# dmjovan/NeRF-Workspaces-Explorer

Measured on AMD Instinct MI355X. Metric: ray-samples/sec (800x800, 192 samples, 8x256 MLP), higher is better.
Workload: dtype f16x3 (split-fp16 MFMA, fp32 accumulate)

## Files before the change

include/nwe.h:

```cpp
#ifndef NWE_H
#define NWE_H

#include <stdint.h>

#ifdef __cplusplus
extern "C" {
#endif

typedef struct nwe_ctx nwe_ctx;

enum {
    NWE_OK = 0,
    NWE_ERR_INVALID = 1,
    NWE_ERR_UNSUPPORTED = 2,
    NWE_ERR_HIP = 3,
    NWE_ERR_STATE = 4
};

enum { NWE_NET_COARSE = 0, NWE_NET_FINE = 1 };

enum {
    NWE_PREC_F16X3 = 0,
    NWE_PREC_F16X1 = 1,
    NWE_PREC_F32 = 2
// ... 60 lines not shown

int nwe_to8b(nwe_ctx *ctx, const float *rgb_dev, uint8_t *out_dev, int64_t n, void *stream);

int64_t nwe_flops_per_eval(const nwe_ctx *ctx, int which);

float nwe_last_kernel_ms(nwe_ctx *ctx);

int nwe_last_launch_parts(nwe_ctx *ctx, float *ms2, int64_t *rays2);


int64_t nwe_packed_bytes(const nwe_ctx *ctx, int which);
int nwe_packed_copy(const nwe_ctx *ctx, int which, void *host_dst, int64_t bytes);
int64_t nwe_packed_bias_count(const nwe_ctx *ctx, int which);
int nwe_packed_bias_copy(const nwe_ctx *ctx, int which, float *host_dst, int64_t count);
float nwe_packed_scale(const nwe_ctx *ctx, int which);

int nwe_debug_set_fine_depths(nwe_ctx *ctx, const float *z_dev);

int nwe_debug_set_raw(nwe_ctx *ctx, const float *raw_coarse_dev, const float *raw_fine_dev);
int nwe_debug_set_coarse_weights(nwe_ctx *ctx, const float *weights_dev);

int nwe_debug_set_fold(nwe_ctx *ctx, int on);

int nwe_set_white_background(nwe_ctx *ctx, int on);

int nwe_set_train_tables(nwe_ctx *ctx, const float *t_rand_dev, const float *noise_coarse_dev, const float *noise_fine_dev,
                         const float *u_sorted_dev);

int nwe_debug_set_decomposition(nwe_ctx *ctx, int mode);
int nwe_debug_last_plan(const nwe_ctx *ctx);
// ... 10 lines not shown
```

nerf-workspaces-explorer_amd/_lib.py:

```python
from __future__ import annotations

import ctypes as C
import os

_HERE = os.path.dirname(os.path.abspath(__file__))
LIB_PATH = os.environ.get("NWE_LIB") or os.path.join(_HERE, "libnwe_hip.so")

NWE_OK, NWE_ERR_INVALID, NWE_ERR_UNSUPPORTED, NWE_ERR_HIP, NWE_ERR_STATE = 0, 1, 2, 3, 4
NET_COARSE, NET_FINE = 0, 1
PREC_F16X3, PREC_F16X1, PREC_F32 = 0, 1, 2
PRECISIONS = {"f16x3": PREC_F16X3, "f16x1": PREC_F16X1, "f32": PREC_F32}

OUTPUT_FIELDS = ("rgb", "depth", "acc", "disp", "z_std", "rgb_coarse", "depth_coarse", "acc_coarse", "disp_coarse",
                 "raw_coarse", "raw_fine", "z_fine", "weights_coarse", "sample_cond", "sample_amp", "sample_switch", "feat_map", "flags")

SYMBOLS = ("nwe_create", "nwe_destroy", "nwe_last_error", "nwe_set_network", "nwe_set_sampling", "nwe_render", "nwe_render_tiled",
           "nwe_create_rays", "nwe_render_rays", "nwe_to8b", "nwe_flops_per_eval", "nwe_last_kernel_ms", "nwe_packed_bytes",
           "nwe_packed_copy", "nwe_packed_bias_count", "nwe_packed_bias_copy", "nwe_packed_scale",
           "nwe_debug_set_fine_depths", "nwe_debug_set_raw", "nwe_debug_set_coarse_weights", "nwe_debug_set_fold", "nwe_set_train_tables", "nwe_set_white_background", "nwe_debug_set_decomposition", "nwe_debug_last_plan", "nwe_debug_set_stamps", "nwe_selftest",
           "nwe_last_warning", "nwe_debug_peer_access", "nwe_set_network_no_view_dirs", "nwe_last_launch_parts")


class Outputs(C.Structure):
    _fields_ = [("struct_bytes", C.c_uint64)] + [(name, C.c_void_p) for name in OUTPUT_FIELDS]

    def __init__(self, **kw):
        super().__init__(struct_bytes=C.sizeof(Outputs), **kw)


_lib = None


def build_hint() -> str:
# ... 17 lines not shown
        "nwe_set_network_no_view_dirs": (I, [P, I, I, I, I, I, I, C.POINTER(P), C.POINTER(P)]),
        "nwe_set_sampling": (I, [P, P, P, I, P, I]),
        "nwe_render": (I, [P, P, I, I, I, F, F, F, F, F, F, I, I, I, C.POINTER(Outputs), P]),
        "nwe_render_tiled": (I, [C.POINTER(P), I, P, I, I, I, F, F, F, F, F, F, I, P, P, P, P, P]),
        "nwe_create_rays": (I, [P, P, I, I, I, F, F, F, F, F, F, I, I, P, P]),
        "nwe_render_rays": (I, [P, P, I64, I, C.POINTER(Outputs), P]),
        "nwe_to8b": (I, [P, P, P, I64, P]),
        "nwe_flops_per_eval": (I64, [P, I]),
        "nwe_last_kernel_ms": (F, [P]),
        "nwe_last_launch_parts": (I, [P, C.POINTER(F), C.POINTER(I64)]),
        "nwe_packed_bytes": (I64, [P, I]),
        "nwe_packed_copy": (I, [P, I, P, I64]),
        "nwe_packed_bias_count": (I64, [P, I]),
        "nwe_packed_bias_copy": (I, [P, I, P, I64]),
        "nwe_packed_scale": (F, [P, I]),
        "nwe_debug_set_fine_depths": (I, [P, P]),
        "nwe_debug_set_raw": (I, [P, P, P]),
        "nwe_debug_set_coarse_weights": (I, [P, P]),
        "nwe_debug_set_fold": (I, [P, I]),
        "nwe_set_train_tables": (I, [P, P, P, P, P]),
        "nwe_set_white_background": (I, [P, I]),
        "nwe_debug_set_decomposition": (I, [P, I]),
        "nwe_debug_last_plan": (I, [P]),
        "nwe_debug_set_stamps": (I, [P, P]),
        "nwe_selftest": (I, [P, C.POINTER(C.c_int32)]),
        "nwe_last_warning": (C.c_char_p, [P]),
        "nwe_debug_peer_access": (I, [P, P]),
    }
    for name, (res, args) in sig.items():
        fn = getattr(lib, name)
# ... 4 lines not shown
```

nerf-workspaces-explorer_amd/csrc/nwe_abi.hip:

```cpp
#include <algorithm>
#include <cmath>
#include <cstdlib>
#include <cstring>
#include <string>
#include <vector>

#include "nwe_host.h"

using namespace nwe;

namespace {

struct NetState {
    bool set = false;
    int D = 0, W = 0, in_xyz = 0, in_dir = 0, skip = -1;
    int out_ch = 0;
    int64_t flops = 0;
    std::vector<float> blob;
    NetF32 f32 = {};
    float* d_blob = nullptr;
    bool mfma_ok = false;
    int form = kFormFolded;
    std::vector<uint8_t> stream;
    std::vector<float> bias_tab;
    int n_chunks = 0;
    float w_scale = 1.f;
    NetMfma mf = {};
    uint8_t* d_stream = nullptr;
    float* d_bias = nullptr;
};

thread_local std::string g_create_error;

}

struct nwe_ctx {
    int device = -1;
    bool host_only = false;
    NetState net[2];
    float *d_t = nullptr, *d_omt = nullptr, *d_u = nullptr;
    int ns = 0, ni = 0;
// ... 103 lines not shown
}

template <class T>
void put_chunk(NetState& n, const T* w, const T* b, int ld, const RowMap& rows, int rt, const std::vector<Segment>& segs) {
    for (int i = 0; i < 32; ++i) { const int r = rows(rt, i); n.bias_tab.push_back(r >= 0 ? (float)b[r] : 0.f); }
    for (const Segment& sg : segs)
        for (int s = 0; s < sg.ksteps; ++s) put_tile_pair(n.stream, w, ld, rows, rt, sg, s, n.w_scale);
}

void pack_mfma(NetState& n, const float* const* w, const float* const* b) {
    const int D = n.D, W = n.W, KH = W / 16;
    const int iv = D, ife = D + 1, ia = D + 2, irgb = D + 3;
    const bool folded = n.form == kFormFolded, noview = n.form == kFormNoViewDirs;
    n.stream.clear();
    n.bias_tab.clear();
    std::vector<double> wv, bv;
    if (folded) {
        const int ldv = W + n.in_dir;
        wv.assign((size_t)(W / 2) * ldv, 0.0);
        bv.assign(W / 2, 0.0);
        for (int r = 0; r < W / 2; ++r) {
            const float* vr = w[iv] + (size_t)r * ldv;
            double* o = wv.data() + (size_t)r * ldv;
            double acc_b = (double)b[iv][r];
            for (int k = 0; k < W; ++k) {
                const double vk = (double)vr[k];
                const float* fr = w[ife] + (size_t)k * W;
                for (int c = 0; c < W; ++c) o[c] += vk * (double)fr[c];
                acc_b += vk * (double)b[ife][k];
            }
// ... 19 lines not shown
    };
    layer(0, W, n.in_xyz, W / 32, 0, {{1, 4, 0}});
    for (int i = 1; i < D; ++i) {
        if (i == n.skip + 1) layer(i, W, W + n.in_xyz, W / 32, 0, {{1, 4, 0}, {0, KH, n.in_xyz}});
        else layer(i, W, W, W / 32, 0, {{0, KH, 0}});
    }
    if (noview) {
        layer(D, 4, W, 1, 1, {{0, KH, 0}});
        n.n_chunks = (int)(n.bias_tab.size() / 32);
        return;
    }
    if (!folded) {
        layer(ife, W, W, W / 32, 0, {{0, KH, 0}});
        layer(ia, 1, W, 1, 1, {{0, KH, 0}});
    }
    if (folded) {
        RowMap rows{W / 2, 0};
        for (int rt = 0; rt < W / 64; ++rt) put_chunk(n, wv.data(), bv.data(), W + n.in_dir, rows, rt, {{0, KH, 0}, {2, 2, W}});
    } else {
        layer(iv, W / 2, W + n.in_dir, W / 64, 0, {{0, KH, 0}, {2, 2, W}});
    }
    layer(irgb, 3, W / 2, 1, 1, {{0, KH / 2, 0}});
    n.n_chunks = (int)(n.bias_tab.size() / 32);
    if (folded) {
        for (int k = 0; k < W; ++k) n.bias_tab.push_back(w[ia][k]);
        n.bias_tab.push_back(b[ia][0]);
        n.bias_tab.resize(n.bias_tab.size() + 31, 0.f);
    }
}

void pack_f32(NetState& n, const float* const* w, const float* const* b) {
    n.blob.clear();
    auto add = [&](int li, int K, int N) {
        LayerF32 L; L.K = K; L.N = N; L.wt_off = (int64_t)n.blob.size();
        n.blob.resize(n.blob.size() + (size_t)K * N);
        float* wt = n.blob.data() + L.wt_off;
        for (int k = 0; k < K; ++k) for (int o = 0; o < N; ++o) wt[(size_t)k * N + o] = w[li][(size_t)o * K + k];
        L.b_off = (int64_t)n.blob.size();
        n.blob.insert(n.blob.end(), b[li], b[li] + N);
// ... 208 lines not shown
    for (int i = 0; i < n_layers; ++i)
        if (!w[i] || !b[i]) return fail(c, NWE_ERR_INVALID, "null weight or bias pointer");
    NetState& n = c->net[which];
    n.set = false;
    n.D = depth; n.W = width; n.in_xyz = in_xyz; n.in_dir = in_dir; n.skip = skip_layer; n.out_ch = out_ch;
    n.flops = algo_flops(n);
    pack_f32(n, w, b);
    n.form = in_dir == 0 ? kFormNoViewDirs : (c->fold != 0 ? kFormFolded : kFormReference);
    n.mfma_ok = mfma_supported(depth, width, in_xyz, in_dir, skip_layer, n.form);
    if (n.mfma_ok) pack_mfma(n, w, b); else { n.stream.clear(); n.bias_tab.clear(); n.n_chunks = 0; }
    n.mf = {};
    n.mf.D = depth; n.mf.W = width; n.mf.skip = skip_layer; n.mf.form = n.form;
    n.mf.n_tiles = (int)(n.stream.size() / kTileBytes);
    n.mf.n_chunks = n.mfma_ok ? n.n_chunks : 0;
    n.mf.inv_scale = 1.f / n.w_scale;
    if (!c->host_only) {
        DeviceGuard guard;
        HIPCHK(c, hipSetDevice(c->device));
        { const int rc = wait_for_launches(c); if (rc) return rc; }
        if (n.d_blob) { (void)hipFree(n.d_blob); n.d_blob = nullptr; }
        if (n.d_stream) { (void)hipFree(n.d_stream); n.d_stream = nullptr; }
        if (n.d_bias) { (void)hipFree(n.d_bias); n.d_bias = nullptr; }
        HIPCHK(c, hipMalloc(&n.d_blob, n.blob.size() * sizeof(float)));
        HIPCHK(c, hipMemcpy(n.d_blob, n.blob.data(), n.blob.size() * sizeof(float), hipMemcpyHostToDevice));
        if (n.mfma_ok) {
            HIPCHK(c, hipMalloc(&n.d_stream, n.stream.size()));
            HIPCHK(c, hipMemcpy(n.d_stream, n.stream.data(), n.stream.size(), hipMemcpyHostToDevice));
            HIPCHK(c, hipMalloc(&n.d_bias, n.bias_tab.size() * sizeof(float)));
            HIPCHK(c, hipMemcpy(n.d_bias, n.bias_tab.data(), n.bias_tab.size() * sizeof(float), hipMemcpyHostToDevice));
        }
// ... 291 lines not shown
    return (int64_t)c->net[which].bias_tab.size();
}

int nwe_packed_bias_copy(const nwe_ctx* c, int which, float* host_dst, int64_t count) {
    if (!c || which < 0 || which > 1 || !host_dst || !c->net[which].set) return NWE_ERR_INVALID;
    if (count != (int64_t)c->net[which].bias_tab.size()) return NWE_ERR_INVALID;
    std::memcpy(host_dst, c->net[which].bias_tab.data(), (size_t)count * sizeof(float));
    return NWE_OK;
}

float nwe_packed_scale(const nwe_ctx* c, int which) {
    if (!c || which < 0 || which > 1 || !c->net[which].set) return 0.f;
    return c->net[which].w_scale;
}

int nwe_debug_set_fine_depths(nwe_ctx* c, const float* z_dev) {
    if (!c) return NWE_ERR_INVALID;
    c->dbg_z_fine = z_dev;
    return NWE_OK;
}

int nwe_debug_set_raw(nwe_ctx* c, const float* raw_coarse_dev, const float* raw_fine_dev) {
    if (!c) return NWE_ERR_INVALID;
    c->dbg_raw_c = raw_coarse_dev; c->dbg_raw_f = raw_fine_dev;
    return NWE_OK;
}

int nwe_debug_set_coarse_weights(nwe_ctx* c, const float* weights_dev) {
    if (!c) return NWE_ERR_INVALID;
    c->dbg_w = weights_dev;
// ... 59 lines not shown
```

nerf-workspaces-explorer_amd/csrc/nwe_host.h:

```cpp
#pragma once
#include <hip/hip_runtime.h>
#include <stdint.h>

#include "nwe_device.h"

namespace nwe {

struct LayerF32 {
    int K, N;
    int64_t wt_off, b_off;
};
struct NetF32 {
    const float* blob;
    int D, W, in_xyz, in_dir, skip;
    LayerF32 pts[16];
    LayerF32 views, feature, alpha, rgb;
    LayerF32 output;
    int out_ch;
};
constexpr int kMaxDepth = 16;

void launch_render_f32(const RenderArgs& a, const NetF32& nc, const NetF32& nf, hipStream_t stream);

struct NetMfma {
    const uint8_t* stream;
    const float* bias;
    int n_tiles, n_chunks;
    float inv_scale;
    int D, W, skip;
    int form;
};

enum Form {
    kFormReference = 0,
    kFormFolded = 1,
    kFormNoViewDirs = 2
};

bool mfma_supported(int D, int W, int in_xyz, int in_dir, int skip, int form);
struct LaunchInfo {
    hipEvent_t mid = nullptr;
    int plan = -1;
    int64_t rays_first = 0;
    bool mid_recorded = false;
};
// ... 10 lines not shown
```

nerf-workspaces-explorer_amd/csrc/nwe_mfma_kernels.h:

```cpp
#pragma once
#include "nwe_host.h"

namespace nwe {

typedef _Float16 h8 __attribute__((ext_vector_type(8)));
typedef float f16v __attribute__((ext_vector_type(16)));

#define LDS_AS __attribute__((address_space(3)))

constexpr int kWaves = 4;
constexpr int kRaysPerWave = 32;

template <int W, int D>
struct Shape {
    static constexpr int NT = W / 32;
    static constexpr int KH = W / 16;
    static constexpr int KG = 4;
    static constexpr int KD = 2;
    static constexpr int NTV = W / 64;
    static constexpr int KV = W / 32;
    static constexpr int N_L0 = 2 * KG / kWaves;
    static constexpr int N_H = 2 * KH / kWaves;
    static constexpr int N_S = 2 * (KH + KG) / kWaves;
    static constexpr int N_V = 2 * (KH + KD) / kWaves;
// ... 189 lines not shown
    const char* buf0;
    const char* tail0;
    int t3;
    uint32_t blk_dst_tail;
    int tail_first;
    const float* bias_tab;
    int chunk;
    int b;
    int wave;
    uint32_t lane_off;
    const uint8_t* blk_src;
    uint32_t blk_dst;
    bool skip_lo = false;
#ifdef NWE_STAMPS
    unsigned long long st_pre = 0, st_wait = 0, st_post = 0, st_t0 = 0;
#endif

    __device__ __forceinline__ void start(const uint8_t* s, const float* bias) {
        stream = s; bias_tab = bias; next_tile = 0; chunk = 0; b = 0; t3 = 0;
    }
    __device__ __forceinline__ const char* cur() const { return buf0 + b * CHUNK_BYTES; }
    __device__ __forceinline__ const char* next() const { return buf0 + (b ^ 1) * CHUNK_BYTES; }
    __device__ __forceinline__ const char* tail() const { return tail0 + t3 * (2 * kTileBytes); }
    __device__ __forceinline__ void begin(int n_per_wave, int buffer, int ahead) {
        blk_src = stream + ((size_t)next_tile + (size_t)wave * n_per_wave) * kTileBytes;
        blk_dst = lds_chunks + buffer * CHUNK_BYTES + wave * n_per_wave * kTileBytes;
        next_tile += n_per_wave * kWaves;
        skip_lo = !X3 && (n_per_wave & 1) == 0;
        if (X3) {
            int slot = t3 + ahead;
// ... 346 lines not shown
            const _Float16 hh = (_Float16)v;
            Ehi[s][j] = hh;
            Elo[s][j] = X3 ? (_Float16)(v - (float)hh) : (_Float16)0.f;
        }
    }
}

template <int W, int D, bool X3>
struct ViewDma {
    using S = Shape<W, D>;
    static constexpr int nb(int rt) { return rt + 1 < S::NTV ? S::N_V : S::N_RGB; }
    static constexpr int na(int rt) { return rt + 2 < S::NTV ? S::N_V : (rt + 2 == S::NTV ? S::N_RGB : 0); }
    using Plan0 = EpiPlan<X3, S::KH, S::KH + S::KD, true, DmaPlan<nb(0), na(0), S::KH + S::KD>::mask()>;
};

template <int RT, int W, int D, bool X3, bool SIGMA_TILE, class WalkerT>
__device__ __forceinline__ void view_tiles(WalkerT& wk, Frags& F, int lane, h8* Ahi, h8* Alo, const h8* GDhi,
                                           const h8* GDlo, h8* Bhi, h8* Blo, Pend& P0, Pend& P1, float inv_scale,
                                           const float* dot_tab = nullptr, float* dot = nullptr) {
    using S = Shape<W, D>;
    constexpr int par = SIGMA_TILE ? (RT + 1) & 1 : RT & 1;
    Pend& cur = par ? P1 : P0;
    Pend& prev = par ? P0 : P1;
    constexpr int PH = (RT * (S::KH + S::KD)) % (PD + 1);
    constexpr int NB = ViewDma<W, D, X3>::nb(RT);
    constexpr int NA = ViewDma<W, D, X3>::na(RT);
    if constexpr (RT == 0 && SIGMA_TILE) {
        h8 d0, d1, d2, d3;
        tile_mma<0, S::KH, S::KD, PH, X3, false, NB, NA, true>(wk, F, lane, false, false, false, nullptr, nullptr, Ahi, Alo, GDhi, GDlo, cur,
                                                               prev, inv_scale, 0.f, d0, d1, d2, d3);
    } else if constexpr (RT == 0) {
        constexpr int L = 2 * S::NT - 2;
        tile_mma<0, S::KH, S::KD, PH, X3, true, NB, NA, true, true, true>(wk, F, lane, false, false, false, nullptr, nullptr, Ahi, Alo, GDhi, GDlo,
                                                                          cur, prev, inv_scale, 0.f, Ahi[L], Alo[L], Ahi[L + 1], Alo[L + 1], -1,
                                                                          dot_tab + (S::NT - 1) * 32, dot);
    } else {
        tile_mma<0, S::KH, S::KD, PH, X3, true, NB, NA, true>(wk, F, lane, false, false, false, nullptr, nullptr, Ahi, Alo, GDhi, GDlo, cur,
                                                              prev, inv_scale, 0.f, Bhi[2 * RT - 2], Blo[2 * RT - 2], Bhi[2 * RT - 1],
                                                              Blo[2 * RT - 1]);
    }
    if constexpr (RT + 1 < S::NTV) view_tiles<RT + 1, W, D, X3, SIGMA_TILE>(wk, F, lane, Ahi, Alo, GDhi, GDlo, Bhi, Blo, P0, P1, inv_scale);
}

#ifndef NWE_COARSE_DENSITY_ONLY
#define NWE_COARSE_DENSITY_ONLY 1
#endif
template <int D, int SKIP>
constexpr bool density_only_built(int form) {
    return NWE_COARSE_DENSITY_ONLY != 0 && form == kFormFolded && !(SKIP >= 0 && SKIP / 2 == D / 2 - 1);
}

template <int W, int D, int SKIP, bool X3, int FORM, class WalkerT>
__device__ __forceinline__ void mlp_eval(WalkerT& wk, Frags& F, int lane, float inv_scale, h8* Ghi, h8* Glo, const char* gd_lds,
                                         const float* dot_tab, bool density_only, float& o_r, float& o_g, float& o_b, float& o_s) {
    using S = Shape<W, D>;
    static_assert(D % 2 == 0, "trunk depth must be even");
    static_assert(SKIP < 0 || SKIP % 2 == 0, "skip layer index must be even");
    static_assert(S::NT % 2 == 0 && S::NTV % 2 == 0, "tile counts must be even");
    constexpr bool FOLD = FORM == kFormFolded, NOVIEW = FORM == kFormNoViewDirs;
    h8 Ahi[S::KH], Alo[S::KH], Bhi[S::KH], Blo[S::KH];
    Pend P0, P1;
    constexpr int NPAIR = D / 2;
    constexpr int SKIP_PAIR = SKIP < 0 ? -1 : SKIP / 2;

    layer<S::NT, 0, S::KG, X3, false, S::N_H, true>(wk, F, lane, false, SKIP_PAIR == 0, nullptr, nullptr, Ghi, Glo, Ahi, Alo, P0, P1,
                                                    inv_scale, 0.f, 0.f);
    auto pair_body = [&](bool use_g, bool skip_next, bool last) __attribute__((always_inline)) {
        layer<S::NT, S::KG, S::KH, X3, true, S::N_H, false>(wk, F, lane, use_g, false, Ghi, Glo, Ahi, Alo, Bhi, Blo, P0, P1, inv_scale,
                                                            0.f, 0.f);
// ... 7 lines not shown
#endif
    if constexpr (NWE_PEEL_SKIP != 0 && SKIP_PAIR >= 0 && SKIP_PAIR < PAIRS) {
#pragma unroll 1
        for (int pair = 0; pair < SKIP_PAIR; ++pair) pair_body(false, pair + 1 == SKIP_PAIR, false);
        pair_body(true, false, SKIP_PAIR == NPAIR - 1);
#pragma unroll 1
        for (int pair = SKIP_PAIR + 1; pair < PAIRS; ++pair) pair_body(false, false, pair == NPAIR - 1);
    } else {
#pragma unroll 1
        for (int pair = 0; pair < PAIRS; ++pair) {
            const bool last = pair == NPAIR - 1;
            pair_body(pair == SKIP_PAIR, !last && pair + 1 == SKIP_PAIR, last);
        }
    }
    float sig = 0.f;
    auto sigma_of = [&]() __attribute__((always_inline)) { return __fadd_rn(__fadd_rn(sig, __shfl_xor(sig, 32, 64)), dot_tab[S::NT * 32]); };
    if constexpr (FOLD) {
        constexpr bool G_LAST = SKIP_PAIR == NPAIR - 1;
        if constexpr (density_only_built<D, SKIP>(FORM)) {
            if (density_only) {
                using TrunkA = EpiPlan<X3, S::KH, S::KH, false, DmaPlan<S::N_H, S::N_V, S::KH>::mask()>;
                using TrunkA0 = EpiPlan<X3, S::KH, S::KH, false, DmaPlan<S::N_H, 0, S::KH>::mask()>;
                using TrunkB = EpiPlan<X3, S::KH, S::KH, false, DmaPlan<S::N_V, S::N_V, S::KH>::mask()>;
                using TrunkB0 = EpiPlan<X3, S::KH, S::KH, false, DmaPlan<0, 0, S::KH>::mask()>;
                static_assert(TrunkA::NG == TrunkA0::NG && TrunkB::NG == TrunkB0::NG,
                              "the last trunk tiles must run the epilogues they carry in the full evaluation's order (dot FMAs)");
                static_assert(!G_LAST, "density_only_built: the last trunk layer takes no gamma(x) k-steps here");
                layer<S::NT, 0, S::KH, X3, true, 0, false, true, 0, false>(wk, F, lane, false, false, nullptr, nullptr, Ahi, Alo, Bhi, Blo, P0, P1,
                                                                           inv_scale, 0.f, 0.f, -1, dot_tab, &sig);
                drain_dot<typename ViewDma<W, D, X3>::Plan0, X3>(P1, inv_scale, dot_tab + (S::NT - 1) * 32 + 4 * (lane >> 5), sig);
                o_s = sigma_of();
// ... 14 lines not shown
                                                              P1, inv_scale, 0.f, Bhi[L], Blo[L], Bhi[L + 1], Blo[L + 1]);
        o_r = pend_value(P0, 0, inv_scale);
        o_g = pend_value(P0, 1, inv_scale);
        o_b = pend_value(P0, 2, inv_scale);
        o_s = pend_value(P0, 3, inv_scale);
        return;
    }
    static_assert((S::NTV * (S::KH + S::KD)) % (PD + 1) == 0, "the view tiles must restore the ring phase");
    h8 GDhi[S::KD], GDlo[S::KD];
#pragma unroll
    for (int k = 0; k < S::KD; ++k) {
        GDhi[k] = *reinterpret_cast<const h8*>(gd_lds + (2 * k) * kTileBytes);
        if (X3) GDlo[k] = *reinterpret_cast<const h8*>(gd_lds + (2 * k + 1) * kTileBytes);
    }
    if constexpr (FOLD) {
        view_tiles<0, W, D, X3, false>(wk, F, lane, Bhi, Blo, GDhi, GDlo, Ahi, Alo, P0, P1, inv_scale, dot_tab, &sig);
        const float sigma = sigma_of();
        tile_mma<0, S::KV, 0, 0, X3, true, 0, 0, false, true>(wk, F, lane, false, false, false, nullptr, nullptr, Ahi, Alo, nullptr, nullptr, P0,
                                                              P1, inv_scale, 0.f, Ahi[LV], Alo[LV], Ahi[LV + 1], Alo[LV + 1]);
        o_s = sigma;
        o_r = pend_value(P0, 0, inv_scale);
        o_g = pend_value(P0, 1, inv_scale);
        o_b = pend_value(P0, 2, inv_scale);
        return;
    } else {
        tile_mma<0, S::KH, 0, 0, X3, true, S::N_V, S::N_V, true>(wk, F, lane, false, false, false, nullptr, nullptr, Bhi, Blo, nullptr, nullptr,
                                                                 P0, P1, inv_scale, -INFINITY, Ahi[L], Alo[L], Ahi[L + 1], Alo[L + 1]);
        const float sigma = pend_value(P0, 0, inv_scale);
        view_tiles<0, W, D, X3, true>(wk, F, lane, Ahi, Alo, GDhi, GDlo, Bhi, Blo, P0, P1, inv_scale);
        tile_mma<0, S::KV, 0, 0, X3, true, 0, 0, false, true>(wk, F, lane, false, false, false, nullptr, nullptr, Bhi, Blo, nullptr, nullptr, P1,
                                                              P0, inv_scale, 0.f, Bhi[LV], Blo[LV], Bhi[LV + 1], Blo[LV + 1]);
        o_s = sigma;
// ... 10 lines not shown
struct Smem {
    using S = Shape<W, D>;
    static constexpr int WBYTES = (SPLIT ? kSplitMaxSamples : kWaves * kPacketMaxSamples) * kRaysPerWave * 4;
    static constexpr int CHUNKS = 2 * S::CHUNK_BYTES;
    static constexpr int BOFF = CHUNKS;
    static constexpr int BIAS_BYTES = ((S::N_CHUNKS * 32 * 4 + 255) / 256) * 256;
    static constexpr int WOFF = BOFF + 2 * BIAS_BYTES;
    static constexpr int TOFF = WOFF + WBYTES;
    static constexpr int XOFF = TOFF + (2 * kMaxSamples + kMaxImportance) * 4;
    static constexpr int LOFF = XOFF + (SPLIT ? 2 * kWaves * kRaysPerWave * 16 : 0);
    static constexpr int GOFF = LOFF + 3 * 2 * kTileBytes;
    static constexpr int TOTAL = GOFF + kWaves * 2 * S::KD * kTileBytes;
    static_assert(XOFF % 16 == 0 && LOFF % 16 == 0 && GOFF % 16 == 0 && TOTAL <= 160 * 1024, "LDS budget");
};

__host__ __device__ inline bool is_lean(const RenderArgs& a) {
    const nwe_outputs& o = a.out;
    return !o.raw_coarse && !o.raw_fine && !o.z_fine && !o.weights_coarse && !o.disp && !o.z_std && !o.rgb_coarse && !o.depth_coarse &&
           !o.acc_coarse && !o.disp_coarse && !o.sample_cond && !o.sample_amp && !o.sample_switch && !o.feat_map && !a.z_fine_in && !a.raw_in_c &&
           !a.raw_in_f && !a.w_in && !a.t_rand && !a.noise_c && !a.noise_f && !a.u_rand && !a.stamps && !a.rays;
}

template <int W, int D, int SKIP, bool X3, bool SPLIT, int FORM, bool LEAN>
__global__ void __launch_bounds__(256) render_mfma_kernel(RenderArgs a_in, NetMfma nc, NetMfma nf) {
    RenderArgs a = a_in;
    if constexpr (LEAN) {
        a.out.raw_coarse = a.out.raw_fine = a.out.z_fine = a.out.weights_coarse = nullptr;
        a.out.disp = a.out.z_std = a.out.rgb_coarse = a.out.depth_coarse = a.out.acc_coarse = a.out.disp_coarse = nullptr;
        a.out.sample_cond = a.out.sample_amp = a.out.sample_switch = a.out.feat_map = nullptr;
        a.z_fine_in = a.raw_in_c = a.raw_in_f = a.w_in = a.t_rand = a.noise_c = a.noise_f = a.u_rand = nullptr;
        a.stamps = nullptr; a.rays = nullptr;
    }
    using S = Shape<W, D>;
    using SM = Smem<W, D, SPLIT>;
    __shared__ __attribute__((aligned(16))) char smem[SM::TOTAL];

    const int lane = threadIdx.x & 63;
    const int wave = __builtin_amdgcn_readfirstlane(threadIdx.x >> 6);
    const int half = lane >> 5;
    const int ns = a.n_samples, ni = a.n_importance;
// ... 19 lines not shown
    const int row = (int)(ridx64 < a.n_rays ? ridx64 : a.n_rays - 1);
    const int64_t ridx = row, rclamp = row;
    const RaySeed seed = seed_ray(a, rclamp);
    auto fresh_ray = [&]() __attribute__((always_inline)) {
        RaySeed sd = seed;
        asm volatile("" : "+v"(sd.pose), "+v"(sd.x), "+v"(sd.y));
        return make_ray<false>(a, sd);
    };

    Walker<S::CHUNK_BYTES, X3> wk;
    wk.buf0 = smem; wk.lds_chunks = (uint32_t)(uintptr_t)(LDS_AS char*)smem;
    wk.tail0 = smem + SM::LOFF; wk.lds_tail = wk.lds_chunks + SM::LOFF; wk.t3 = 0;
    wk.b = 0; wk.wave = wave; wk.lane_off = lane * 16;

    char* gd_lds = smem + SM::GOFF + wave * (2 * S::KD * kTileBytes) + lane * 16;
    if constexpr (FORM != kFormNoViewDirs) {
        const Ray rv = make_ray<true>(a, seed);
        h8 GDhi[S::KD], GDlo[S::KD];
        encode<2, S::KD, X3>(rv.vx, rv.vy, rv.vz, half, GDhi, GDlo);
#pragma unroll
        for (int k = 0; k < S::KD; ++k) {
            *reinterpret_cast<h8*>(gd_lds + (2 * k) * kTileBytes) = GDhi[k];
            *reinterpret_cast<h8*>(gd_lds + (2 * k + 1) * kTileBytes) = GDlo[k];
        }
    }

    FineSampler fs;
    fs.wc = reinterpret_cast<float*>(smem + SM::WOFF) + (SPLIT ? 0 : wave * (kPacketMaxSamples * kRaysPerWave)) + (lane & 31);
    const bool wc_writer = !SPLIT || wave == 0;
    fs.stride = kRaysPerWave; fs.u_tab = s_u; fs.ns = ns; fs.ni = ni;
    fs.cd.t_tab = s_t; fs.cd.omt_tab = s_omt; fs.cd.ns = ns;
    fs.cd.jitter = a.t_rand; fs.cd.row = row;
    fs.u_rand = a.u_rand;
    __syncthreads();

    Composite comp;
    uint32_t flags = 0;
#ifdef NWE_STAMPS
    unsigned long long st_enc = 0, st_sync = 0, st_mlp = 0, st_comp = 0;
    const unsigned long long st_begin = __builtin_amdgcn_s_memtime();
    const unsigned long long st_real = __builtin_amdgcn_s_memrealtime();
#endif
    for (int pass = 0; pass < (ni > 0 ? 2 : 1); ++pass) {
        const NetMfma& net = pass == 0 ? nc : nf;
        const float* bias = s_bias + (pass == 0 ? 0 : SM::BIAS_BYTES / 4);
        const float* dot_tab = bias + NCH * 32;
        const int Stot = pass == 0 ? ns : ns + ni;
        const bool density_only = LEAN && density_only_built<D, SKIP>(FORM) && pass == 0 && ni > 0;
        const float* noise = pass == 0 ? a.noise_c : a.noise_f;
        const float* raw_in = pass == 0 ? a.raw_in_c : a.raw_in_f;
        if (pass == 0 && a.w_in) {
            if (wc_writer) for (int s = 0; s < ns; ++s) fs.wc[s * kRaysPerWave] = a.w_in[rclamp * ns + s];
            continue;
        }
        comp.reset();
        if constexpr (SPLIT) {
            int produced = 0;
            auto gen = [&](const Ray& ray) -> float {
                const int i = produced++;
                if (i >= Stot) return 0.f;
                if (pass == 0) return fs.cd.z(ray, i);
                return a.z_fine_in ? a.z_fine_in[rclamp * Stot + i] : fs.next(ray);
            };
// ... 71 lines not shown
                wk.template sync<false>();
                Frags F;
#pragma unroll
                for (int k = 0; k < PD; ++k) {
                    F.hi[k] = *reinterpret_cast<const h8*>(wk.cur() + lane * 16 + (2 * k) * kTileBytes);
                    if (X3) F.lo[k] = *reinterpret_cast<const h8*>(wk.cur() + lane * 16 + (2 * k + 1) * kTileBytes);
                }
                if (it > 0) drain(it - 1);
#pragma unroll
                for (int k = 0; k < 4; ++k) zp[k] = zq[k];
#ifdef NWE_STAMPS
                const unsigned long long t2 = __builtin_amdgcn_s_memtime();
                wk.st_t0 = t2;
                st_sync += t2 - t1;
#endif
                mlp_eval<W, D, SKIP, X3, FORM>(wk, F, lane, net.inv_scale, Ghi, Glo, gd_lds, dot_tab, density_only, rr, rg, rb, rs);
#ifdef NWE_STAMPS
                st_mlp += __builtin_amdgcn_s_memtime() - t2;
#endif
                }
#ifdef NWE_STAMPS
                const unsigned long long t3 = __builtin_amdgcn_s_memtime();
#endif
                if (own_valid) {
                    xch[(it & 1) * (kWaves * kRaysPerWave) + wave * kRaysPerWave + (lane & 31)] =
                        Composite::shade(rr, rg, rb, rs, z_own, z_nxt, s_own + 1 == Stot, ray.dnorm, noise ? noise[rclamp * Stot + s_own] : 0.f);
                    if (lane_live) {
                        float* raw = pass == 0 ? a.out.raw_coarse : a.out.raw_fine;
                        if (raw) {
                            *reinterpret_cast<float4*>(raw + (ridx * Stot + s_own) * 4) = make_float4(rr, rg, rb, rs);
                            if (bad(rr) || bad(rg) || bad(rb) || bad(rs)) flags |= NWE_FLAG_RAW;
// ... 56 lines not shown
                const unsigned long long t1 = __builtin_amdgcn_s_memtime();
                st_enc += t1 - t0;
    #endif
                wk.template sync<false>();
                Frags F;
    #pragma unroll
                for (int k = 0; k < PD; ++k) {
                    F.hi[k] = *reinterpret_cast<const h8*>(wk.cur() + lane * 16 + (2 * k) * kTileBytes);
                    if (X3) F.lo[k] = *reinterpret_cast<const h8*>(wk.cur() + lane * 16 + (2 * k + 1) * kTileBytes);
                }
    #ifdef NWE_STAMPS
                const unsigned long long t2 = __builtin_amdgcn_s_memtime();
                wk.st_t0 = t2;
                st_sync += t2 - t1;
    #endif
                mlp_eval<W, D, SKIP, X3, FORM>(wk, F, lane, net.inv_scale, Ghi, Glo, gd_lds, dot_tab, density_only, rr, rg, rb, rs);
    #ifdef NWE_STAMPS
                st_mlp += __builtin_amdgcn_s_memtime() - t2;
    #endif
                }
    #ifdef NWE_STAMPS
                const unsigned long long t3 = __builtin_amdgcn_s_memtime();
    #endif
                const float w = comp.step(rr, rg, rb, rs, z_cur, z_next, s + 1 == Stot, ray.dnorm, noise ? noise[rclamp * Stot + s] : 0.f);
                if (pass == 0) fs.wc[s * kRaysPerWave] = w;
                if (lane_live) {
                    if (pass == 0 && a.out.weights_coarse) a.out.weights_coarse[ridx * ns + s] = w;
                    float* raw = pass == 0 ? a.out.raw_coarse : a.out.raw_fine;
                    if (raw) {
                        *reinterpret_cast<float4*>(raw + (ridx * Stot + s) * 4) = make_float4(rr, rg, rb, rs);
                        if (bad(rr) || bad(rg) || bad(rb) || bad(rs)) flags |= NWE_FLAG_RAW;
// ... 5 lines not shown
                st_comp += __builtin_amdgcn_s_memtime() - t3;
    #endif
            }
        }
        if (live) {
            flags |= store_ray(a.out, ridx, comp, pass == 1, a.white_bkgd != 0) & (density_only ? ~(uint32_t)NWE_FLAG_RGB_COARSE : ~0u);
            if (ni == 0) flags |= store_ray(a.out, ridx, comp, true, a.white_bkgd != 0);
        }
    }
    if (flags && a.out.flags) atomicOr(a.out.flags, flags);
#ifdef NWE_STAMPS
    if (a.stamps && lane == 0) {
        unsigned long long* o = a.stamps + ((size_t)blockIdx.x * kWaves + wave) * 10;
        o[0] = st_enc; o[1] = st_sync; o[2] = st_mlp; o[3] = st_comp; o[4] = __builtin_amdgcn_s_memtime() - st_begin;
        o[5] = wk.st_pre; o[6] = wk.st_wait; o[7] = wk.st_post;
        o[8] = __builtin_amdgcn_s_memrealtime() - st_real; o[9] = st_begin;
    }
#endif
}

template <int W, int D, int SKIP, int FORM>
inline void launch_one(RenderArgs a, const NetMfma& nc, const NetMfma& nf, bool three_pass, bool split, int64_t ray_first, int64_t rays,
                       hipStream_t stream) {
    if (rays <= 0) return;
    a.ray_first = ray_first;
    const int64_t per_wg = split ? kRaysPerWave : kWaves * kRaysPerWave;
    const unsigned blocks = (unsigned)((rays + per_wg - 1) / per_wg);
#define NWE_LAUNCH(X3_, SPLIT_, LEAN_) \
    hipLaunchKernelGGL((render_mfma_kernel<W, D, SKIP, X3_, SPLIT_, FORM, LEAN_>), dim3(blocks), dim3(256), 0, stream, a, nc, nf)
    const bool lean = is_lean(a);
    if (three_pass) {
// ... 44 lines not shown
```

nerf-workspaces-explorer_amd/renderer.py:

```python
from __future__ import annotations

import ctypes as C
from typing import Dict, Iterable, Mapping, Optional, Sequence, Tuple

import numpy as np
import torch

from . import _lib

LAYER_ORDER_TAIL = ("_views_linears.0", "_feature_linear", "_alpha_linear", "_rgb_linear")

_PER_RAY = {"rgb": 3, "depth": 1, "acc": 1, "disp": 1, "z_std": 1, "rgb_coarse": 3, "depth_coarse": 1,
            "acc_coarse": 1, "disp_coarse": 1, "sample_cond": 1, "sample_amp": 1, "sample_switch": 1}


def normalize_state_dict(sd: Mapping[str, object]) -> Dict[str, np.ndarray]:
    out = {}
    for k, v in sd.items():
        if isinstance(v, torch.Tensor):
            v = v.detach().cpu().numpy()
        v = np.ascontiguousarray(np.asarray(v, dtype=np.float32))
        out[k if k.startswith("_") else "_" + k] = v
    return out

# ... 265 lines not shown
            rc = self._lib.nwe_packed_copy(self._ctx, which, buf.ctypes.data, n)
            if rc != _lib.NWE_OK:
                raise RuntimeError("nwe_packed_copy failed")
        return buf

    def packed_bias(self, which: int) -> np.ndarray:
        n = int(self._lib.nwe_packed_bias_count(self._ctx, which))
        buf = np.empty(n, dtype=np.float32)
        if n and self._lib.nwe_packed_bias_copy(self._ctx, which, buf.ctypes.data, n) != _lib.NWE_OK:
            raise RuntimeError("nwe_packed_bias_copy failed")
        return buf.reshape(-1, 32)

    def packed_scale(self, which: int) -> float:
        return float(self._lib.nwe_packed_scale(self._ctx, which))

    def selftest(self):
        rep = (C.c_int32 * 8)()
        rc = self._lib.nwe_selftest(self._ctx, rep)
        return rc, list(rep)


class TiledRenderer:

    def __init__(self, devices: Sequence[int]):
        if not devices:
            raise ValueError("TiledRenderer needs at least one device")
        self.parts = [Renderer(int(d)) for d in devices]
        self.devices = [int(d) for d in devices]
        self._lib = self.parts[0]._lib
        self._ctxs = (C.c_void_p * len(self.parts))(*[p._ctx for p in self.parts])
# ... 56 lines not shown
```

Measured before the change: 347.3 million.

## Skip colour-branch MFMA tiles when every lane's density is non-positive

Adds a wave-uniform check after the density output: if every sample in the wave has sigma <= 0 (so its alpha is zero after ReLU), the remaining view/colour tiles are not computed and only their weight-stream DMA is drained to keep the walker pipeline consistent. The skip is guarded by host-side finiteness checks of the packed colour weights and device-side finiteness checks of the direction encoding, so that NaN/Inf propagation semantics are preserved. It aims to cut MFMA work for empty space in the fine pass, at the cost of an extra ballot and branch plus code size and register pressure. The hollow DMA walk must stay exactly in step with the real tile schedule.

```diff
diff --git a/include/nwe.h b/include/nwe.h
--- a/include/nwe.h
+++ b/include/nwe.h
@@ -98,6 +98,7 @@
 int64_t nwe_packed_bias_count(const nwe_ctx *ctx, int which);
 int nwe_packed_bias_copy(const nwe_ctx *ctx, int which, float *host_dst, int64_t count);
 float nwe_packed_scale(const nwe_ctx *ctx, int which);
+int nwe_packed_colour_finite(const nwe_ctx *ctx, int which);
 
 int nwe_debug_set_fine_depths(nwe_ctx *ctx, const float *z_dev);
 
diff --git a/nerf-workspaces-explorer_amd/_lib.py b/nerf-workspaces-explorer_amd/_lib.py
--- a/nerf-workspaces-explorer_amd/_lib.py
+++ b/nerf-workspaces-explorer_amd/_lib.py
@@ -16,7 +16,7 @@
 
 SYMBOLS = ("nwe_create", "nwe_destroy", "nwe_last_error", "nwe_set_network", "nwe_set_sampling", "nwe_render", "nwe_render_tiled",
            "nwe_create_rays", "nwe_render_rays", "nwe_to8b", "nwe_flops_per_eval", "nwe_last_kernel_ms", "nwe_packed_bytes",
-           "nwe_packed_copy", "nwe_packed_bias_count", "nwe_packed_bias_copy", "nwe_packed_scale",
+           "nwe_packed_copy", "nwe_packed_bias_count", "nwe_packed_bias_copy", "nwe_packed_scale", "nwe_packed_colour_finite",
            "nwe_debug_set_fine_depths", "nwe_debug_set_raw", "nwe_debug_set_coarse_weights", "nwe_debug_set_fold", "nwe_set_train_tables", "nwe_set_white_background", "nwe_debug_set_decomposition", "nwe_debug_last_plan", "nwe_debug_set_stamps", "nwe_selftest",
            "nwe_last_warning", "nwe_debug_peer_access", "nwe_set_network_no_view_dirs", "nwe_last_launch_parts")
 
@@ -64,6 +64,7 @@
         "nwe_packed_bias_count": (I64, [P, I]),
         "nwe_packed_bias_copy": (I, [P, I, P, I64]),
         "nwe_packed_scale": (F, [P, I]),
+        "nwe_packed_colour_finite": (I, [P, I]),
         "nwe_debug_set_fine_depths": (I, [P, P]),
         "nwe_debug_set_raw": (I, [P, P, P]),
         "nwe_debug_set_coarse_weights": (I, [P, P]),
diff --git a/nerf-workspaces-explorer_amd/csrc/nwe_abi.hip b/nerf-workspaces-explorer_amd/csrc/nwe_abi.hip
--- a/nerf-workspaces-explorer_amd/csrc/nwe_abi.hip
+++ b/nerf-workspaces-explorer_amd/csrc/nwe_abi.hip
@@ -25,6 +25,7 @@
     std::vector<float> bias_tab;
     int n_chunks = 0;
     float w_scale = 1.f;
+    bool colour_finite = false;
     NetMfma mf = {};
     uint8_t* d_stream = nullptr;
     float* d_bias = nullptr;
@@ -158,6 +159,7 @@
     const bool folded = n.form == kFormFolded, noview = n.form == kFormNoViewDirs;
     n.stream.clear();
     n.bias_tab.clear();
+    n.colour_finite = false;
     std::vector<double> wv, bv;
     if (folded) {
         const int ldv = W + n.in_dir;
@@ -207,6 +209,7 @@
         layer(ife, W, W, W / 32, 0, {{0, KH, 0}});
         layer(ia, 1, W, 1, 1, {{0, KH, 0}});
     }
+    const size_t colour_stream = n.stream.size(), colour_bias = n.bias_tab.size();
     if (folded) {
         RowMap rows{W / 2, 0};
         for (int rt = 0; rt < W / 64; ++rt) put_chunk(n, wv.data(), bv.data(), W + n.in_dir, rows, rt, {{0, KH, 0}, {2, 2, W}});
@@ -216,6 +219,11 @@
     layer(irgb, 3, W / 2, 1, 1, {{0, KH / 2, 0}});
     n.n_chunks = (int)(n.bias_tab.size() / 32);
     if (folded) {
+        bool finite = true;
+        const _Float16* hp = reinterpret_cast<const _Float16*>(n.stream.data() + colour_stream);
+        for (size_t k = 0; k < (n.stream.size() - colour_stream) / sizeof(_Float16); ++k) finite = finite && std::isfinite((float)hp[k]);
+        for (size_t k = colour_bias; k < n.bias_tab.size(); ++k) finite = finite && std::isfinite(n.bias_tab[k]);
+        n.colour_finite = finite;
         for (int k = 0; k < W; ++k) n.bias_tab.push_back(w[ia][k]);
         n.bias_tab.push_back(b[ia][0]);
         n.bias_tab.resize(n.bias_tab.size() + 31, 0.f);
@@ -454,6 +462,7 @@
     n.mf.n_tiles = (int)(n.stream.size() / kTileBytes);
     n.mf.n_chunks = n.mfma_ok ? n.n_chunks : 0;
     n.mf.inv_scale = 1.f / n.w_scale;
+    n.mf.colour_finite = (n.mfma_ok && n.form == kFormFolded && n.colour_finite) ? 1 : 0;
     if (!c->host_only) {
         DeviceGuard guard;
         HIPCHK(c, hipSetDevice(c->device));
@@ -775,6 +784,11 @@
     return c->net[which].w_scale;
 }
 
+int nwe_packed_colour_finite(const nwe_ctx* c, int which) {
+    if (!c || which < 0 || which > 1 || !c->net[which].set) return 0;
+    return c->net[which].mf.colour_finite;
+}
+
 int nwe_debug_set_fine_depths(nwe_ctx* c, const float* z_dev) {
     if (!c) return NWE_ERR_INVALID;
     c->dbg_z_fine = z_dev;
diff --git a/nerf-workspaces-explorer_amd/csrc/nwe_host.h b/nerf-workspaces-explorer_amd/csrc/nwe_host.h
--- a/nerf-workspaces-explorer_amd/csrc/nwe_host.h
+++ b/nerf-workspaces-explorer_amd/csrc/nwe_host.h
@@ -29,6 +29,7 @@
     float inv_scale;
     int D, W, skip;
     int form;
+    int colour_finite;
 };
 
 enum Form {
diff --git a/nerf-workspaces-explorer_amd/csrc/nwe_mfma_kernels.h b/nerf-workspaces-explorer_amd/csrc/nwe_mfma_kernels.h
--- a/nerf-workspaces-explorer_amd/csrc/nwe_mfma_kernels.h
+++ b/nerf-workspaces-explorer_amd/csrc/nwe_mfma_kernels.h
@@ -227,6 +227,7 @@
     bool skip_lo = false;
 #ifdef NWE_STAMPS
     unsigned long long st_pre = 0, st_wait = 0, st_post = 0, st_t0 = 0;
+    unsigned long long st_skipped = 0;
 #endif
 
     __device__ __forceinline__ void start(const uint8_t* s, const float* bias) {
@@ -603,7 +604,7 @@
     using Plan0 = EpiPlan<X3, S::KH, S::KH + S::KD, true, DmaPlan<nb(0), na(0), S::KH + S::KD>::mask()>;
 };
 
-template <int RT, int W, int D, bool X3, bool SIGMA_TILE, class WalkerT>
+template <int RT, int W, int D, bool X3, bool SIGMA_TILE, bool ONLY = false, class WalkerT>
 __device__ __forceinline__ void view_tiles(WalkerT& wk, Frags& F, int lane, h8* Ahi, h8* Alo, const h8* GDhi,
                                            const h8* GDlo, h8* Bhi, h8* Blo, Pend& P0, Pend& P1, float inv_scale,
                                            const float* dot_tab = nullptr, float* dot = nullptr) {
@@ -628,7 +629,7 @@
                                                               prev, inv_scale, 0.f, Bhi[2 * RT - 2], Blo[2 * RT - 2], Bhi[2 * RT - 1],
                                                               Blo[2 * RT - 1]);
     }
-    if constexpr (RT + 1 < S::NTV) view_tiles<RT + 1, W, D, X3, SIGMA_TILE>(wk, F, lane, Ahi, Alo, GDhi, GDlo, Bhi, Blo, P0, P1, inv_scale);
+    if constexpr (!ONLY && RT + 1 < S::NTV) view_tiles<RT + 1, W, D, X3, SIGMA_TILE>(wk, F, lane, Ahi, Alo, GDhi, GDlo, Bhi, Blo, P0, P1, inv_scale);
 }
 
 #ifndef NWE_COARSE_DENSITY_ONLY
@@ -639,9 +640,43 @@
     return NWE_COARSE_DENSITY_ONLY != 0 && form == kFormFolded && !(SKIP >= 0 && SKIP / 2 == D / 2 - 1);
 }
 
-template <int W, int D, int SKIP, bool X3, int FORM, class WalkerT>
+#ifndef NWE_SKIP_DEAD_COLOUR
+#define NWE_SKIP_DEAD_COLOUR 1
+#endif
+#ifndef NWE_DEAD_COLOUR_AT
+#define NWE_DEAD_COLOUR_AT 1
+#endif
+template <int D, int SKIP>
+constexpr bool dead_colour_built(int form) {
+    return NWE_SKIP_DEAD_COLOUR != 0 && form == kFormFolded;
+}
+
+template <int NQ, int NB, int NA, class WalkerT>
+__device__ __forceinline__ void hollow_tile(WalkerT& wk) {
+    using DP = DmaPlan<NB, NA, NQ>;
+    static_for<0, DP::REST>([&](auto jc) __attribute__((always_inline)) { wk.piece(PD + decltype(jc)::value, NB >= 8  ? NB - 2 : -1); });
+    wk.template sync<false>();
+    if constexpr (NA > 0) {
+        wk.begin(NA, wk.b, 2);
+        static_for<0, (NA < PD ? NA : PD)>([&](auto ic) __attribute__((always_inline)) { wk.piece(decltype(ic)::value); });
+    }
+    wk.tile_done();
+}
+
+template <int RT, int W, int D, bool X3, class WalkerT>
+__device__ __forceinline__ void hollow_colour(WalkerT& wk) {
+    using S = Shape<W, D>;
+    if constexpr (RT < S::NTV) {
+        hollow_tile<S::KH + S::KD, ViewDma<W, D, X3>::nb(RT), ViewDma<W, D, X3>::na(RT)>(wk);
+        hollow_colour<RT + 1, W, D, X3>(wk);
+    } else {
+        hollow_tile<S::KV, 0, 0>(wk);
+    }
+}
+
+template <int W, int D, int SKIP, bool X3, int FORM, bool DEAD = false, class WalkerT>
 __device__ __forceinline__ void mlp_eval(WalkerT& wk, Frags& F, int lane, float inv_scale, h8* Ghi, h8* Glo, const char* gd_lds,
-                                         const float* dot_tab, bool density_only, float& o_r, float& o_g, float& o_b, float& o_s) {
+                                         const float* dot_tab, bool density_only, bool may_skip, float& o_r, float& o_g, float& o_b, float& o_s) {
     using S = Shape<W, D>;
     static_assert(D % 2 == 0, "trunk depth must be even");
     static_assert(SKIP < 0 || SKIP % 2 == 0, "skip layer index must be even");
@@ -679,7 +714,9 @@
         }
     }
     float sig = 0.f;
-    auto sigma_of = [&]() __attribute__((always_inline)) { return __fadd_rn(__fadd_rn(sig, __shfl_xor(sig, 32, 64)), dot_tab[S::NT * 32]); };
+    auto sigma_from = [&](float sg) __attribute__((always_inline)) { return __fadd_rn(__fadd_rn(sg, __shfl_xor(sg, 32, 64)), dot_tab[S::NT * 32]); };
+    auto sigma_of = [&]() __attribute__((always_inline)) { return sigma_from(sig); };
+    auto all_dead = [&](float sigma) __attribute__((always_inline)) { return __ballot(!(sigma <= 0.f && sigma > -INFINITY)) == 0ull; };
     if constexpr (FOLD) {
         constexpr bool G_LAST = SKIP_PAIR == NPAIR - 1;
         if constexpr (density_only_built<D, SKIP>(FORM)) {
@@ -724,8 +761,37 @@
         if (X3) GDlo[k] = *reinterpret_cast<const h8*>(gd_lds + (2 * k + 1) * kTileBytes);
     }
     if constexpr (FOLD) {
-        view_tiles<0, W, D, X3, false>(wk, F, lane, Bhi, Blo, GDhi, GDlo, Ahi, Alo, P0, P1, inv_scale, dot_tab, &sig);
+        if constexpr (DEAD && NWE_DEAD_COLOUR_AT == 0) {
+            if (may_skip) {
+                float sig2 = sig;
+                drain_dot<typename ViewDma<W, D, X3>::Plan0, X3>(P1, inv_scale, dot_tab + (S::NT - 1) * 32 + 4 * (lane >> 5), sig2);
+                const float sigma2 = sigma_from(sig2);
+                if (all_dead(sigma2)) {
+                    hollow_colour<0, W, D, X3>(wk);
+#ifdef NWE_STAMPS
+                    ++wk.st_skipped;
+#endif
+                    o_s = sigma2;
+                    o_r = o_g = o_b = 0.f;
+                    return;
+                }
+            }
+        }
+        constexpr bool LATE = DEAD && NWE_DEAD_COLOUR_AT != 0;
+        view_tiles<0, W, D, X3, false, LATE>(wk, F, lane, Bhi, Blo, GDhi, GDlo, Ahi, Alo, P0, P1, inv_scale, dot_tab, &sig);
         const float sigma = sigma_of();
+        if constexpr (LATE) {
+            if (may_skip && all_dead(sigma)) {
+                hollow_colour<1, W, D, X3>(wk);
+#ifdef NWE_STAMPS
+                ++wk.st_skipped;
+#endif
+                o_s = sigma;
+                o_r = o_g = o_b = 0.f;
+                return;
+            }
+            view_tiles<1, W, D, X3, false>(wk, F, lane, Bhi, Blo, GDhi, GDlo, Ahi, Alo, P0, P1, inv_scale);
+        }
         tile_mma<0, S::KV, 0, 0, X3, true, 0, 0, false, true>(wk, F, lane, false, false, false, nullptr, nullptr, Ahi, Alo, nullptr, nullptr, P0,
                                                               P1, inv_scale, 0.f, Ahi[LV], Alo[LV], Ahi[LV + 1], Alo[LV + 1]);
         o_s = sigma;
@@ -766,16 +832,23 @@
     static_assert(XOFF % 16 == 0 && LOFF % 16 == 0 && GOFF % 16 == 0 && TOTAL <= 160 * 1024, "LDS budget");
 };
 
-__host__ __device__ inline bool is_lean(const RenderArgs& a) {
+__host__ __device__ inline bool is_lean(const RenderArgs& a, bool ignore_stamps = false) {
     const nwe_outputs& o = a.out;
     return !o.raw_coarse && !o.raw_fine && !o.z_fine && !o.weights_coarse && !o.disp && !o.z_std && !o.rgb_coarse && !o.depth_coarse &&
            !o.acc_coarse && !o.disp_coarse && !o.sample_cond && !o.sample_amp && !o.sample_switch && !o.feat_map && !a.z_fine_in && !a.raw_in_c &&
-           !a.raw_in_f && !a.w_in && !a.t_rand && !a.noise_c && !a.noise_f && !a.u_rand && !a.stamps && !a.rays;
+           !a.raw_in_f && !a.w_in && !a.t_rand && !a.noise_c && !a.noise_f && !a.u_rand && (ignore_stamps || !a.stamps) && !a.rays;
 }
 
 template <int W, int D, int SKIP, bool X3, bool SPLIT, int FORM, bool LEAN>
 __global__ void __launch_bounds__(256) render_mfma_kernel(RenderArgs a_in, NetMfma nc, NetMfma nf) {
     RenderArgs a = a_in;
+#ifdef NWE_STAMPS
+    constexpr bool DEAD = dead_colour_built<D, SKIP>(FORM);
+    const bool dead_frame = LEAN || is_lean(a_in, true);
+#else
+    constexpr bool DEAD = LEAN && dead_colour_built<D, SKIP>(FORM);
+    constexpr bool dead_frame = true;
+#endif
     if constexpr (LEAN) {
         a.out.raw_coarse = a.out.raw_fine = a.out.z_fine = a.out.weights_coarse = nullptr;
         a.out.disp = a.out.z_std = a.out.rgb_coarse = a.out.depth_coarse = a.out.acc_coarse = a.out.disp_coarse = nullptr;
@@ -825,6 +898,7 @@
     wk.b = 0; wk.wave = wave; wk.lane_off = lane * 16;
 
     char* gd_lds = smem + SM::GOFF + wave * (2 * S::KD * kTileBytes) + lane * 16;
+    bool gd_finite = false;
     if constexpr (FORM != kFormNoViewDirs) {
         const Ray rv = make_ray<true>(a, seed);
         h8 GDhi[S::KD], GDlo[S::KD];
@@ -833,6 +907,17 @@
         for (int k = 0; k < S::KD; ++k) {
             *reinterpret_cast<h8*>(gd_lds + (2 * k) * kTileBytes) = GDhi[k];
             *reinterpret_cast<h8*>(gd_lds + (2 * k + 1) * kTileBytes) = GDlo[k];
+        }
+        if constexpr (DEAD) {
+            typedef uint32_t u4 __attribute__((ext_vector_type(4)));
+            uint32_t nonfinite = 0;
+#pragma unroll
+            for (int k = 0; k < 2 * S::KD; ++k) {
+                const u4 v = __builtin_bit_cast(u4, k < S::KD ? GDhi[k] : GDlo[k - S::KD]);
+#pragma unroll
+                for (int j = 0; j < 4; ++j) nonfinite |= (uint32_t)((v[j] & 0x7c00u) == 0x7c00u) | (uint32_t)((v[j] & 0x7c000000u) == 0x7c000000u);
+            }
+            gd_finite = __ballot(nonfinite != 0) == 0ull;
         }
     }
 
@@ -858,6 +943,7 @@
         const float* dot_tab = bias + NCH * 32;
         const int Stot = pass == 0 ? ns : ns + ni;
         const bool density_only = LEAN && density_only_built<D, SKIP>(FORM) && pass == 0 && ni > 0;
+        const bool may_skip = DEAD && dead_frame && gd_finite && net.colour_finite != 0 && (pass == 1 || ni == 0);
         const float* noise = pass == 0 ? a.noise_c : a.noise_f;
         const float* raw_in = pass == 0 ? a.raw_in_c : a.raw_in_f;
         if (pass == 0 && a.w_in) {
@@ -959,7 +1045,7 @@
                 wk.st_t0 = t2;
                 st_sync += t2 - t1;
 #endif
-                mlp_eval<W, D, SKIP, X3, FORM>(wk, F, lane, net.inv_scale, Ghi, Glo, gd_lds, dot_tab, density_only, rr, rg, rb, rs);
+                mlp_eval<W, D, SKIP, X3, FORM, DEAD>(wk, F, lane, net.inv_scale, Ghi, Glo, gd_lds, dot_tab, density_only, may_skip, rr, rg, rb, rs);
 #ifdef NWE_STAMPS
                 st_mlp += __builtin_amdgcn_s_memtime() - t2;
 #endif
@@ -1046,7 +1132,7 @@
                 wk.st_t0 = t2;
                 st_sync += t2 - t1;
     #endif
-                mlp_eval<W, D, SKIP, X3, FORM>(wk, F, lane, net.inv_scale, Ghi, Glo, gd_lds, dot_tab, density_only, rr, rg, rb, rs);
+                mlp_eval<W, D, SKIP, X3, FORM, DEAD>(wk, F, lane, net.inv_scale, Ghi, Glo, gd_lds, dot_tab, density_only, may_skip, rr, rg, rb, rs);
     #ifdef NWE_STAMPS
                 st_mlp += __builtin_amdgcn_s_memtime() - t2;
     #endif
@@ -1082,7 +1168,7 @@
         unsigned long long* o = a.stamps + ((size_t)blockIdx.x * kWaves + wave) * 10;
         o[0] = st_enc; o[1] = st_sync; o[2] = st_mlp; o[3] = st_comp; o[4] = __builtin_amdgcn_s_memtime() - st_begin;
         o[5] = wk.st_pre; o[6] = wk.st_wait; o[7] = wk.st_post;
-        o[8] = __builtin_amdgcn_s_memrealtime() - st_real; o[9] = st_begin;
+        o[8] = __builtin_amdgcn_s_memrealtime() - st_real; o[9] = wk.st_skipped;
     }
 #endif
 }
diff --git a/nerf-workspaces-explorer_amd/renderer.py b/nerf-workspaces-explorer_amd/renderer.py
--- a/nerf-workspaces-explorer_amd/renderer.py
+++ b/nerf-workspaces-explorer_amd/renderer.py
@@ -303,6 +303,9 @@
     def packed_scale(self, which: int) -> float:
         return float(self._lib.nwe_packed_scale(self._ctx, which))
 
+    def packed_colour_finite(self, which: int) -> bool:
+        return bool(self._lib.nwe_packed_colour_finite(self._ctx, which))
+
     def selftest(self):
         rep = (C.c_int32 * 8)()
         rc = self._lib.nwe_selftest(self._ctx, rep)
```

After: 350.4 million, median of 6. About the same (+0.9%).
